# rafifmalikdzaki/Multitask-Bonetumor-yolo

Measured on AMD Instinct MI355X. Metric: images/sec at 640x640 multitask fwd (det+seg+cls) + decode/NMS/masks, higher is better.
Workload: dtype bf16; 1 GPU; configs[1]: batch-16/GPU 640x640 multitask inference (ConvNeXt-T + C2f-BiFPN + Detect/Segment/cls) + decode + per-image NMS(top-100) + mask assembly; random-init weights; batch_per_gpu=16, img=640, parallelism=dp1 (batch sharded, no data-path collective)

## Files before the change

### include/mtbt_hip.h

```cpp
#ifndef MTBT_HIP_H
#define MTBT_HIP_H

#include <stdint.h>

#ifdef __cplusplus
extern "C" {
#endif

#define MTBT_OK 0
#define MTBT_EINVAL (-1)
#define MTBT_EALIGN (-2)
#define MTBT_ELAUNCH (-3)
#define MTBT_EWORKSPACE (-4)

#define MTBT_F32 0
#define MTBT_BF16 1
#define MTBT_F16 2

#define MTBT_ACT_NONE 0
#define MTBT_ACT_SILU 1
#define MTBT_ACT_ELU 2
#define MTBT_ACT_GELU 3
#define MTBT_ACT_DSILU 5
#define MTBT_ACT_DELU 6
// ... 104 lines not shown
  int32_t act1;
  int32_t act2;
} mtbt_pw_chain_args;
int mtbt_pw_chain_nhwc(const mtbt_pw_chain_args* a, void* stream);
int mtbt_pw_chain_supported(const mtbt_pw_chain_args* a);
int mtbt_sizeof_pw_chain_args(void);

int64_t mtbt_bn_train_workspace_bytes(int64_t pixels, int C);
int mtbt_bn_train_nhwc(const void* x, void* y, const float* gamma, const float* beta, float* running_mean,
                       float* running_var, float momentum, float eps, int act, int64_t pixels, int C, int dtype,
                       void* workspace, int64_t workspace_bytes, void* stream);

int mtbt_gap_fc(const void* x, const float* w, const float* b, float* y, int N, int HW, int C,
                int nout, int dtype, void* stream);

typedef struct mtbt_decode_args {
  const float* map[3];
  int32_t h[3], w[3];
  int32_t map_pixel_stride[3];
  float stride[3];
  int32_t n_levels, N, nc, reg_max;
  int32_t xywh;
  float* boxes;
  float* scores;
  float* best_score;
  int32_t* best_label;
  float* preds_cat;
  int32_t cat_stride;
} mtbt_decode_args;

int mtbt_decode_boxes(const mtbt_decode_args* a, void* stream);

int64_t mtbt_nms_workspace_bytes(int N, int A);
int mtbt_nms_batched(const float* boxes, const float* best_score, const int32_t* best_label, int N, int A,
                     float conf_th, float iou_th, float clamp_max, int top_k, int64_t* keep_idx,
                     int32_t* keep_anchor, float* out_boxes, float* out_scores, int64_t* out_labels,
                     int32_t* counts, int32_t* n_cand, void* workspace, int64_t workspace_bytes,
                     void* stream);

typedef struct mtbt_mask_args {
  const float* protos;
  const float* coeff;
  int64_t coeff_batch_stride, coeff_k_stride, coeff_c_stride;
  const int32_t* gather_idx;
  const int32_t* counts;
  float bias;
  int32_t N, K, nm, hp, wp, Hout, Wout;
  float* logits;
  uint8_t* masks;
} mtbt_mask_args;

int mtbt_mask_assemble(const mtbt_mask_args* a, void* stream);

typedef struct mtbt_frame {
  int32_t height, width;
  float step;
  float scale;
  int32_t pitch;
  int32_t reserved;
  int64_t offset;
} mtbt_frame;

typedef struct mtbt_frame_mask_args {
  const float* protos;
  const float* coeff;
  int64_t coeff_batch_stride, coeff_k_stride, coeff_c_stride;
  const int32_t* gather_idx;
  const int32_t* counts;
  const float* boxes;
  float* boxes_frame;
  uint8_t* out;
  int64_t out_bytes;
  int32_t N, K, nm, hp, wp;
  int32_t crop;
} mtbt_frame_mask_args;

int mtbt_masks_to_frames(const mtbt_frame_mask_args* a, const mtbt_frame* frames, int n_frames, void* stream);
int mtbt_sizeof_frame_args(int which);

#define MTBT_FUSE_MAX_SOURCES 8
#define MTBT_FUSE_MAX_CANDIDATES 4096
typedef struct mtbt_box_fuse_args {
  const float* boxes[MTBT_FUSE_MAX_SOURCES];
  const float* scores[MTBT_FUSE_MAX_SOURCES];
  const int64_t* labels[MTBT_FUSE_MAX_SOURCES];
  const int32_t* counts[MTBT_FUSE_MAX_SOURCES];
  const int32_t* anchors[MTBT_FUSE_MAX_SOURCES];
  int32_t orient[MTBT_FUSE_MAX_SOURCES];
  float weight[MTBT_FUSE_MAX_SOURCES];
  int32_t n_sources, N, K, top_k;
  float img_size, iou_thr, skip_thr;
  int32_t reserved;
  float* out_boxes;
  float* out_scores;
  int64_t* out_labels;
  int32_t* out_counts;
  int32_t* n_clusters;
  int32_t* n_members;
  int32_t* lead_source;
  int32_t* lead_slot;
  int32_t* lead_anchor;
  void* workspace;
  int64_t workspace_bytes;
} mtbt_box_fuse_args;

int64_t mtbt_fuse_workspace_bytes(int n_sources, int N, int K);
// ... 423 lines not shown
```

### multitask_bonetumor_yolo_amd/_lib.py

```python
import ctypes as C
import os

_HERE = os.path.dirname(os.path.abspath(__file__))
LIB_PATH = os.path.join(_HERE, "csrc", "libmtbt_hip.so")

ABI_VERSION = 5
F32, BF16, F16 = 0, 1, 2
ACT_NONE, ACT_SILU, ACT_ELU, ACT_GELU, ACT_GELU_POLY, ACT_DSILU, ACT_DELU, ACT_DGELU, ACT_DGELU_POLY = 0, 1, 2, 3, 4, 5, 6, 7, 8
OUT_NHWC, OUT_CONVT2X2 = 0, 1
RES_ID, RES_UP_BILINEAR, RES_DOWN_MEAN, RES_UP_NEAREST, RES_MAXPOOL = 0, 1, 2, 3, 4
CONFUSION_MAX_NC = 64

ERRORS = {-1: "MTBT_EINVAL (bad argument / unsupported shape)", -2: "MTBT_EALIGN (misaligned pointer or stride)",
          -3: "MTBT_ELAUNCH (kernel launch failed)", -4: "MTBT_EWORKSPACE (workspace too small)"}


class ConvArgs(C.Structure):
    _fields_ = [
        ("x", C.c_void_p), ("w", C.c_void_p), ("y", C.c_void_p), ("scale", C.c_void_p), ("shift", C.c_void_p),
        ("res", C.c_void_p),
        ("x_batch_stride", C.c_int64), ("y_batch_stride", C.c_int64), ("res_batch_stride", C.c_int64),
        ("x_pixel_stride", C.c_int32), ("y_pixel_stride", C.c_int32), ("res_pixel_stride", C.c_int32),
        ("N", C.c_int32), ("H", C.c_int32), ("W", C.c_int32), ("C", C.c_int32), ("K", C.c_int32),
        ("R", C.c_int32), ("S", C.c_int32), ("stride", C.c_int32), ("pad", C.c_int32),
# ... 160 lines not shown


class Tile(C.Structure):
    _fields_ = [("image", C.c_int32), ("pox", C.c_int32), ("poy", C.c_int32),
                ("wx0", C.c_int32), ("wy0", C.c_int32), ("wx1", C.c_int32), ("wy1", C.c_int32),
                ("height", C.c_int32), ("width", C.c_int32), ("reserved", C.c_int32),
                ("step", C.c_float), ("scale", C.c_float), ("fox", C.c_float), ("foy", C.c_float)]


class TileMergeArgs(C.Structure):
    _fields_ = [("boxes", C.c_void_p), ("scores", C.c_void_p), ("labels", C.c_void_p), ("counts", C.c_void_p), ("anchors", C.c_void_p),
                ("tiles", C.POINTER(Tile)), ("tiles_dev", C.c_void_p), ("first", C.POINTER(C.c_int32)),
                ("N", C.c_int32), ("n_tiles", C.c_int32), ("K", C.c_int32), ("top_k", C.c_int32),
                ("metric", C.c_int32), ("class_agnostic", C.c_int32), ("thr", C.c_float), ("skip_thr", C.c_float),
                ("out_boxes", C.c_void_p), ("out_scores", C.c_void_p), ("out_labels", C.c_void_p), ("out_counts", C.c_void_p),
                ("n_members", C.c_void_p), ("lead_tile", C.c_void_p), ("lead_slot", C.c_void_p), ("lead_anchor", C.c_void_p),
                ("member_slot", C.c_void_p), ("n_left", C.c_void_p)]


class TileMaskArgs(C.Structure):
    _fields_ = [("protos", C.c_void_p), ("mc", C.c_void_p),
                ("mc_batch_stride", C.c_int64), ("mc_k_stride", C.c_int64), ("mc_c_stride", C.c_int64),
                ("anchors", C.c_void_p), ("scores", C.c_void_p), ("member_slot", C.c_void_p), ("counts", C.c_void_p), ("boxes", C.c_void_p),
                ("tiles", C.POINTER(Tile)), ("tiles_dev", C.c_void_p), ("first", C.POINTER(C.c_int32)),
                ("W", C.c_void_p), ("Ss", C.c_void_p), ("out", C.c_void_p), ("out_bytes", C.c_int64),
                ("N", C.c_int32), ("n_tiles", C.c_int32), ("K", C.c_int32), ("top_k", C.c_int32), ("Tmax", C.c_int32),
                ("nm", C.c_int32), ("hp", C.c_int32), ("wp", C.c_int32), ("crop", C.c_int32), ("reserved", C.c_int32)]


SYMBOLS = {
    "mtbt_abi_version": (C.c_int, []),
    "mtbt_sizeof_args": (C.c_int, [C.c_int]),
    "mtbt_target_arch": (C.c_char_p, []),
    "mtbt_conv2d_nhwc": (C.c_int, [C.POINTER(ConvArgs), C.c_void_p]),
    "mtbt_convt2x2_conv3x3_nhwc": (C.c_int, [C.POINTER(UpconvArgs), C.c_void_p]),
    "mtbt_stem_conv4x4_ln": (C.c_int, [C.c_void_p] * 5 + [C.c_float, C.c_void_p] + [C.c_int] * 5 + [C.c_void_p]),
    "mtbt_dwconv_nhwc": (C.c_int, [C.c_void_p] * 5 + [C.c_float, C.c_void_p, C.c_void_p, C.c_int, C.c_void_p]
                         + [C.c_int] * 6 + [C.c_void_p]),
    "mtbt_layernorm_nhwc": (C.c_int, [C.c_void_p] * 3 + [C.c_float, C.c_void_p, C.c_int64, C.c_int, C.c_int, C.c_void_p]),
    "mtbt_bifpn_fuse": (C.c_int, [C.POINTER(FuseArgs), C.c_void_p]),
    "mtbt_bifpn_node_nhwc": (C.c_int, [C.POINTER(NodeArgs), C.c_void_p]),
    "mtbt_pw_chain_nhwc": (C.c_int, [C.POINTER(PwChainArgs), C.c_void_p]),
    "mtbt_pw_chain_supported": (C.c_int, [C.POINTER(PwChainArgs)]),
    "mtbt_sizeof_pw_chain_args": (C.c_int, []),
    "mtbt_bn_train_workspace_bytes": (C.c_int64, [C.c_int64, C.c_int]),
    "mtbt_bn_train_nhwc": (C.c_int, [C.c_void_p] * 6 + [C.c_float, C.c_float, C.c_int, C.c_int64, C.c_int, C.c_int, C.c_void_p,
                                      C.c_int64, C.c_void_p]),
    "mtbt_gap_fc": (C.c_int, [C.c_void_p] * 4 + [C.c_int] * 5 + [C.c_void_p]),
    "mtbt_decode_boxes": (C.c_int, [C.POINTER(DecodeArgs), C.c_void_p]),
    "mtbt_nms_workspace_bytes": (C.c_int64, [C.c_int, C.c_int]),
    "mtbt_nms_batched": (C.c_int, [C.c_void_p] * 3 + [C.c_int, C.c_int, C.c_float, C.c_float, C.c_float, C.c_int]
                         + [C.c_void_p] * 8 + [C.c_int64, C.c_void_p]),
    "mtbt_mask_assemble": (C.c_int, [C.POINTER(MaskArgs), C.c_void_p]),
    "mtbt_loss_workspace_bytes": (C.c_int64, [C.c_int, C.c_int, C.c_int64]),
    "mtbt_multitask_loss": (C.c_int, [C.POINTER(LossArgs), C.c_void_p]),
    "mtbt_multitask_loss_grad": (C.c_int, [C.POINTER(LossArgs), C.POINTER(C.c_void_p), C.POINTER(C.c_int32), C.c_void_p, C.c_void_p, C.c_void_p]),
    "mtbt_convnext_mlp_fused": (C.c_int, [C.c_void_p] * 7 + [C.c_int64, C.c_int, C.c_void_p]),
    "mtbt_convnext_mlp_fused_dt": (C.c_int, [C.c_void_p] * 7 + [C.c_int64, C.c_int, C.c_int, C.c_void_p]),
    "mtbt_convnext_mlp_fused_train": (C.c_int, [C.c_void_p] * 8 + [C.c_int64, C.c_int, C.c_void_p]),
    "mtbt_bbox_iou_pairwise": (C.c_int, [C.c_void_p, C.c_int, C.c_void_p, C.c_int, C.c_float, C.c_void_p, C.c_void_p]),
    "mtbt_letterbox_batch": (C.c_int, [C.POINTER(RawImage), C.c_int, C.c_int, C.c_void_p, C.c_void_p, C.POINTER(C.c_double), C.c_void_p]),
    "mtbt_augment_batch": (C.c_int, [C.POINTER(RawImage), C.c_int, C.c_int, C.POINTER(C.c_int32), C.c_int, C.c_void_p, C.c_void_p, C.c_void_p, C.c_void_p]),
    "mtbt_mosaic_batch": (C.c_int, [C.POINTER(RawImage), C.c_int, C.c_int, C.POINTER(C.c_int32), C.c_int, C.POINTER(C.c_int32), C.c_void_p, C.c_void_p, C.c_void_p, C.c_void_p]),
    "mtbt_seg_confusion_workspace_bytes": (C.c_int64, [C.c_int]),
    "mtbt_seg_confusion": (C.c_int, [C.c_void_p, C.c_void_p, C.c_int, C.c_int64, C.c_void_p, C.c_void_p, C.c_void_p, C.c_int64, C.c_void_p]),
    "mtbt_conv_wgrad_workspace_bytes": (C.c_int64, [C.c_int] * 7),
    "mtbt_conv_wgrad": (C.c_int, [C.c_void_p] * 3 + [C.c_int] * 9 + [C.c_int64, C.c_int32, C.c_int64, C.c_int32, C.c_int, C.c_int, C.c_void_p,
                                  C.c_int64, C.c_void_p]),
    "mtbt_conv_wgrad_xact": (C.c_int, [C.c_void_p] * 3 + [C.c_int] * 9 + [C.c_int64, C.c_int32, C.c_int64, C.c_int32, C.c_int, C.c_int, C.c_int, C.c_void_p,
                                       C.c_int64, C.c_void_p]),
    "mtbt_conv_wgrad_bias": (C.c_int, [C.c_void_p] * 4 + [C.c_int] * 9 + [C.c_int64, C.c_int32, C.c_int64, C.c_int32, C.c_int, C.c_int, C.c_void_p,
                                       C.c_int64, C.c_void_p]),
    "mtbt_act_backward": (C.c_int, [C.c_void_p] * 3 + [C.c_int64, C.c_int, C.c_int, C.c_void_p]),
    "mtbt_channel_sum_workspace_bytes": (C.c_int64, [C.c_int64, C.c_int]),
    "mtbt_channel_sum": (C.c_int, [C.c_void_p, C.c_void_p, C.c_int64, C.c_int, C.c_int32, C.c_int32, C.c_int, C.c_void_p, C.c_int, C.c_void_p,
                                   C.c_int64, C.c_void_p]),
    "mtbt_channel_affine2": (C.c_int, [C.c_void_p] * 6 + [C.c_int64, C.c_int, C.c_int, C.c_void_p]),
    "mtbt_layernorm_backward_nhwc": (C.c_int, [C.c_void_p] * 3 + [C.c_float, C.c_void_p, C.c_void_p, C.c_int64, C.c_int, C.c_int, C.c_int, C.c_void_p]),
    "mtbt_layernorm_backward_params_workspace_bytes": (C.c_int64, [C.c_int64, C.c_int]),
    "mtbt_layernorm_backward_params_nhwc": (C.c_int, [C.c_void_p] * 3 + [C.c_float, C.c_void_p, C.c_int64, C.c_int, C.c_int, C.c_int, C.c_void_p, C.c_void_p,
                                                      C.c_int, C.c_void_p, C.c_int64, C.c_void_p]),
    "mtbt_dwconv_wgrad_workspace_bytes": (C.c_int64, [C.c_int] * 5),
    "mtbt_dwconv_wgrad": (C.c_int, [C.c_void_p] * 3 + [C.c_int] * 7 + [C.c_void_p, C.c_int64, C.c_void_p]),
    "mtbt_dwconv_wgrad_bias": (C.c_int, [C.c_void_p] * 4 + [C.c_int] * 7 + [C.c_void_p, C.c_int64, C.c_void_p]),
    "mtbt_adamw_step": (C.c_int, [C.c_void_p] * 4 + [C.c_int64] + [C.c_float] * 5 + [C.c_int64, C.c_void_p, C.c_void_p]),
    "mtbt_sgd_step": (C.c_int, [C.c_void_p] * 3 + [C.c_int64] + [C.c_float] * 4 + [C.c_int, C.c_int64, C.c_void_p, C.c_void_p]),
    "mtbt_adamw_step_ema": (C.c_int, [C.c_void_p] * 5 + [C.c_int64] + [C.c_float] * 5 + [C.c_int64, C.c_void_p, C.c_double, C.c_void_p]),
    "mtbt_sgd_step_ema": (C.c_int, [C.c_void_p] * 4 + [C.c_int64] + [C.c_float] * 4 + [C.c_int, C.c_int64, C.c_void_p, C.c_double, C.c_void_p]),
    "mtbt_ema_update": (C.c_int, [C.c_void_p, C.c_void_p, C.c_int64, C.c_double, C.c_void_p]),
    "mtbt_sumsq_workspace_bytes": (C.c_int64, []),
    "mtbt_sumsq": (C.c_int, [C.c_void_p, C.c_int64, C.c_void_p, C.c_int, C.c_void_p, C.c_int64, C.c_void_p]),
    "mtbt_clip_coef": (C.c_int, [C.c_void_p, C.c_float, C.c_void_p, C.c_void_p, C.c_void_p]),
    "mtbt_stem_conv4x4_ln_train": (C.c_int, [C.c_void_p] * 5 + [C.c_float, C.c_void_p, C.c_void_p] + [C.c_int] * 5 + [C.c_void_p]),
    "mtbt_dwconv_nhwc_train": (C.c_int, [C.c_void_p] * 5 + [C.c_float, C.c_void_p, C.c_void_p, C.c_int, C.c_void_p, C.c_void_p, C.c_void_p]
                               + [C.c_int] * 6 + [C.c_void_p]),
    "mtbt_bn_forward_nhwc": (C.c_int, [C.c_void_p, C.c_void_p, C.c_int32] + [C.c_void_p] * 4 + [C.c_float, C.c_float, C.c_int, C.c_int64, C.c_int, C.c_int,
                                       C.c_int, C.c_void_p, C.c_void_p, C.c_int64, C.c_void_p]),
    "mtbt_bn_forward_sums_nhwc": (C.c_int, [C.c_void_p, C.c_void_p, C.c_int32] + [C.c_void_p] * 4 + [C.c_float, C.c_float, C.c_int, C.c_int64, C.c_int, C.c_int,
                                            C.c_void_p, C.c_void_p, C.c_void_p, C.c_void_p]),
    "mtbt_conv_colsum_workspace_bytes": (C.c_int64, [C.c_int64, C.c_int, C.c_int]),
    "mtbt_conv_colsum_layout": (C.c_int, [C.c_void_p, C.c_void_p, C.c_void_p]),
    "mtbt_conv_kernel_choice": (C.c_int, [C.c_void_p, C.c_void_p]),
    "mtbt_conv2d_nhwc_batch": (C.c_int, [C.c_void_p, C.c_int, C.c_void_p]),
    "mtbt_conv_batch_kernel_choice": (C.c_int, [C.c_void_p, C.c_int, C.c_void_p]),
    "mtbt_dwconv3x3_mult_nhwc": (C.c_int, [C.c_void_p] * 4 + [C.c_int, C.c_void_p] + [C.c_int] * 6 + [C.c_void_p]),
    "mtbt_bn_forward_partials_nhwc": (C.c_int, [C.c_void_p, C.c_void_p, C.c_int32] + [C.c_void_p] * 4 + [C.c_float, C.c_float, C.c_int, C.c_int64, C.c_int, C.c_int,
# ... 96 lines not shown
```

### multitask_bonetumor_yolo_amd/csrc/mask_mfma.hip

```cpp
#include "common.h"

namespace {

struct MaskX4P {
  const float* protos;
  const float* coeff;
  long cbs, cks, ccs;
  const int* gather;
  const int* counts;
  float bias;
  int N, K, hp, wp, Hout, Wout;
  float* logits;
  unsigned char* masks;
  int tiles_x, tiles_y;
  int dbg;
};
#ifdef MTBT_MASK_ABLATION
#define MASK_ABL(p, bit) ((p).dbg & (bit))
#else
#define MASK_ABL(p, bit) 0
#endif

constexpr int NM = 32;
constexpr int PPITCH = NM + 1;

template <int LW, int LH, bool MASKS_ONLY>
__global__ __launch_bounds__(256) void mask_x4_kernel(const MaskX4P p) {
  constexpr int PW = LW + 2, PH = LH + 2;
  constexpr int NPX = PW * PH;
  constexpr int NPXP = (NPX + 15) / 16 * 16;
  constexpr int LPITCH = NPXP + 4;
  constexpr int SEGS = LW / 4;
  extern __shared__ __attribute__((aligned(16))) char smem[];
  float* patch = reinterpret_cast<float*>(smem);
  float* coef = patch + NPXP * PPITCH;
  float* low = coef + 16 * PPITCH;
  const int tid = threadIdx.x, lane = tid & 63, wave = tid >> 6;
  const int n = blockIdx.y;
  const int tx = blockIdx.x % p.tiles_x, ty = blockIdx.x / p.tiles_x;
  const int lx_base = tx * LW - 1, ly_base = ty * LH - 1;
  const int cnt = p.counts ? min(p.counts[n], p.K) : p.K;

  const float* pr = p.protos + (long)n * p.hp * p.wp * NM;
  for (int i = tid; i < NPXP * (NM / 4); i += 256) {
    const int px = i >> 3, c4 = i & 7;
    float4 v = make_float4(0.f, 0.f, 0.f, 0.f);
    if (px < NPX && !MASK_ABL(p, 8)) {
      const int py = px / PW, pxx = px - py * PW;
      const int ly = min(max(ly_base + py, 0), p.hp - 1), lx = min(max(lx_base + pxx, 0), p.wp - 1);
      v = *reinterpret_cast<const float4*>(pr + ((long)ly * p.wp + lx) * NM + c4 * 4);
    }
    float* d = patch + px * PPITCH + c4 * 4;
    d[0] = v.x; d[1] = v.y; d[2] = v.z; d[3] = v.w;
  }

  const int row = tid / SEGS, seg = tid % SEGS;
  const int oy = ty * (4 * LH) + row, ox0 = tx * (4 * LW) + seg * 16;
  const int iy = (row + 2) >> 2;
  const float wy1 = ((row + 2) & 3) * 0.25f + 0.125f, wy0 = 1.0f - wy1;

  float cpre[2];
  auto fetch_coef = [&](int g) {
#pragma unroll
    for (int u = 0; u < 2; ++u) {
      const int i = tid + u * 256, b = i >> 5, c = i & 31;
      float v = 0.f;
      if (g + b < cnt) {
        const long kk = p.gather ? p.gather[(long)n * p.K + g + b] : (g + b);
        v = p.coeff[(long)n * p.cbs + kk * p.cks + c * p.ccs];
      }
      cpre[u] = v;
    }
  };
  if (cnt > 0) fetch_coef(0);
  for (int g0 = 0; g0 < cnt; g0 += 16) {
#pragma unroll
    for (int u = 0; u < 2; ++u) {
      const int i = tid + u * 256;
      coef[(i >> 5) * PPITCH + (i & 31)] = cpre[u];
    }
    __syncthreads();
    if (g0 + 16 < cnt) fetch_coef(g0 + 16);
    {
      float a[8];
#pragma unroll
      for (int ks = 0; ks < 8; ++ks) a[ks] = coef[(lane & 15) * PPITCH + ks * 4 + (lane >> 4)];
      for (int pg = wave; pg < NPXP / 16 && !MASK_ABL(p, 4); pg += 4) {
        f32x4 acc = f32x4{p.bias, p.bias, p.bias, p.bias};
        const float* bp = patch + (pg * 16 + (lane & 15)) * PPITCH + (lane >> 4);
#pragma unroll
        for (int ks = 0; ks < 8; ++ks) acc = __builtin_amdgcn_mfma_f32_16x16x4f32(a[ks], bp[ks * 4], acc, 0, 0, 0);
#pragma unroll
        for (int r = 0; r < 4; ++r) low[(4 * (lane >> 4) + r) * LPITCH + pg * 16 + (lane & 15)] = acc[r];
      }
    }
    __syncthreads();
    if (oy < p.Hout && !MASK_ABL(p, 2)) {
      const int nb = min(16, cnt - g0);
      for (int b = 0; b < nb; ++b) {
        const float* r0 = low + b * LPITCH + iy * PW + seg * 4;
        const float* r1 = r0 + PW;
        float t0[6], t1[6];
#pragma unroll
        for (int c = 0; c < 6; ++c) { t0[c] = r0[c]; t1[c] = r1[c]; }
        const long obase_m = (((long)n * p.K + g0 + b) * p.Hout + oy) * p.Wout + ox0;
        if constexpr (MASKS_ONLY) {
          typedef float f2 __attribute__((ext_vector_type(2)));
          float v[6];
#pragma unroll
          for (int c = 0; c < 6; ++c) v[c] = wy0 * t0[c] + wy1 * t1[c];
          unsigned w[4] = {0u, 0u, 0u, 0u};
          if (MASK_ABL(p, 16)) {
#pragma unroll
            for (int e = 0; e < 16; ++e) {
              const int ix = (e + 2) >> 2;
              const float wx1 = ((e + 2) & 3) * 0.25f + 0.125f, wx0 = 1.0f - wx1;
              const float val = wx0 * v[ix] + wx1 * v[ix + 1];
              w[e >> 2] = __builtin_amdgcn_cvt_pk_u8_f32(fmaf(val, 0x1p100f, -0x1p76f), e & 3, w[e >> 2]);
            }
          } else
#pragma unroll
          for (int e = 0; e < 16; e += 2) {
            const int ix = (e + 2) >> 2;
            const float a1 = ((e + 2) & 3) * 0.25f + 0.125f, b1 = ((e + 3) & 3) * 0.25f + 0.125f;
            const f2 W1 = f2{a1 * 0x1p100f, b1 * 0x1p100f}, W0 = f2{(1.0f - a1) * 0x1p100f, (1.0f - b1) * 0x1p100f};
            f2 d = __builtin_elementwise_fma(W0, f2{v[ix], v[ix]}, f2{-0x1p76f, -0x1p76f});
            d = __builtin_elementwise_fma(W1, f2{v[ix + 1], v[ix + 1]}, d);
            w[e >> 2] = __builtin_amdgcn_cvt_pk_u8_f32(d.x, e & 3, w[e >> 2]);
            w[e >> 2] = __builtin_amdgcn_cvt_pk_u8_f32(d.y, (e + 1) & 3, w[e >> 2]);
          }
          if (!MASK_ABL(p, 1) || (w[0] ^ w[1] ^ w[2] ^ w[3]) == 0x12345679u) *reinterpret_cast<uint4*>(p.masks + obase_m) = uint4{w[0] & 0x01010101u, w[1] & 0x01010101u, w[2] & 0x01010101u, w[3] & 0x01010101u};
          continue;
        }
        float o[16];
#pragma unroll
        for (int e = 0; e < 16; ++e) {
          const int ix = (e + 2) >> 2;
          const float wx1 = ((e + 2) & 3) * 0.25f + 0.125f, wx0 = 1.0f - wx1;
          o[e] = wy0 * (wx0 * t0[ix] + wx1 * t0[ix + 1]) + wy1 * (wx0 * t1[ix] + wx1 * t1[ix + 1]);
        }
        const long obase = (((long)n * p.K + g0 + b) * p.Hout + oy) * p.Wout + ox0;
        if (p.logits) {
#pragma unroll
          for (int e = 0; e < 16; e += 4) *reinterpret_cast<float4*>(p.logits + obase + e) = make_float4(o[e], o[e + 1], o[e + 2], o[e + 3]);
        }
        if (p.masks) {
          unsigned w[4] = {0u, 0u, 0u, 0u};
#pragma unroll
          for (int e = 0; e < 16; ++e) w[e >> 2] |= (o[e] > 5.9604645e-8f ? 1u : 0u) << ((e & 3) * 8);
          *reinterpret_cast<uint4*>(p.masks + obase) = uint4{w[0], w[1], w[2], w[3]};
        }
      }
    }
    __syncthreads();
  }
  if (oy < p.Hout) {
    for (int k = cnt; k < p.K; ++k) {
      const long obase = (((long)n * p.K + k) * p.Hout + oy) * p.Wout + ox0;
      if (p.logits) {
#pragma unroll
        for (int e = 0; e < 16; e += 4) *reinterpret_cast<float4*>(p.logits + obase + e) = make_float4(0.f, 0.f, 0.f, 0.f);
      }
      if (p.masks) *reinterpret_cast<uint4*>(p.masks + obase) = uint4{0u, 0u, 0u, 0u};
    }
  }
}

}

template <int LW, int LH>
static int launch_mask_x4(MaskX4P& p, const mtbt_mask_args* a, hipStream_t stream) {
  static_assert(LW * LH == 256 && (LW / 4) * (4 * LH) == 256, "256 threads: one per (output row, 16-pixel segment)");
  constexpr int NPXP = ((LW + 2) * (LH + 2) + 15) / 16 * 16;
  p.tiles_x = a->Wout / (4 * LW);
  p.tiles_y = (a->Hout + 4 * LH - 1) / (4 * LH);
  const size_t lds = (size_t)(NPXP * PPITCH + 16 * PPITCH + 16 * (NPXP + 4)) * sizeof(float);
  if (!a->logits && a->masks) {
    if (int rc = mtbt_allow_lds(mask_x4_kernel<LW, LH, true>, (int)lds)) return rc;
    hipLaunchKernelGGL((mask_x4_kernel<LW, LH, true>), dim3(p.tiles_x * p.tiles_y, a->N), dim3(256), lds, stream, p);
  } else {
    if (int rc = mtbt_allow_lds(mask_x4_kernel<LW, LH, false>, (int)lds)) return rc;
    hipLaunchKernelGGL((mask_x4_kernel<LW, LH, false>), dim3(p.tiles_x * p.tiles_y, a->N), dim3(256), lds, stream, p);
  }
  MTBT_LAUNCH_CHECK();
  return MTBT_OK;
}

int mtbt_mask_x4_try(const mtbt_mask_args* a, hipStream_t stream) {
  if (a->nm != NM || a->Hout != 4 * a->hp || a->Wout != 4 * a->wp || a->Wout % 64 || a->Hout % 4) return 1;
  MaskX4P p;
  p.protos = a->protos; p.coeff = a->coeff; p.cbs = a->coeff_batch_stride; p.cks = a->coeff_k_stride; p.ccs = a->coeff_c_stride;
  p.gather = a->gather_idx; p.counts = a->counts; p.bias = a->bias;
  p.N = a->N; p.K = a->K; p.hp = a->hp; p.wp = a->wp; p.Hout = a->Hout; p.Wout = a->Wout;
  p.logits = a->logits; p.masks = a->masks;
  p.dbg = 0;
  return a->Wout % 128 == 0 ? launch_mask_x4<32, 8>(p, a, stream) : launch_mask_x4<16, 16>(p, a, stream);
}
```

### multitask_bonetumor_yolo_amd/csrc/postprocess.hip

```cpp
#include "common.h"


namespace {

struct DecodeP {
  const float* map[3];
  int h[3], w[3], ld[3], off[4];
  float stride[3];
  int n_levels, N, nc, reg_max, xywh, A;
  float* boxes;
  float* scores;
  float* best_score;
  int* best_label;
  float* preds_cat;
  int cat_stride;
};

__global__ void decode_kernel(const DecodeP p) {
  const long g = (long)blockIdx.x * 64 + (threadIdx.x >> 2);
  const int side = threadIdx.x & 3;
  const long total = (long)p.N * p.A;
  const bool live = g < total;
  const long gg = live ? g : 0;
  const int n = (int)(gg / p.A), a = (int)(gg - (long)n * p.A);
// ... 452 lines not shown
}

extern "C" int mtbt_decode_boxes(const mtbt_decode_args* a, void* stream) {
  if (!a || a->n_levels < 1 || a->n_levels > 3 || a->N <= 0 || a->nc <= 0 || a->reg_max <= 0 || a->reg_max > 64) return MTBT_EINVAL;
  DecodeP p;
  int A = 0;
  for (int l = 0; l < 3; ++l) {
    p.off[l] = A;
    if (l < a->n_levels) {
      if (!a->map[l] || a->h[l] <= 0 || a->w[l] <= 0 || a->map_pixel_stride[l] < 4 * a->reg_max + a->nc) return MTBT_EINVAL;
      p.map[l] = a->map[l]; p.h[l] = a->h[l]; p.w[l] = a->w[l]; p.ld[l] = a->map_pixel_stride[l]; p.stride[l] = a->stride[l];
      A += a->h[l] * a->w[l];
    } else { p.map[l] = nullptr; p.h[l] = p.w[l] = 1; p.ld[l] = 0; p.stride[l] = 0.f; }
  }
  p.off[3] = A;
  if (a->preds_cat && a->cat_stride < 4 + a->nc) return MTBT_EINVAL;
  p.n_levels = a->n_levels; p.N = a->N; p.nc = a->nc; p.reg_max = a->reg_max; p.xywh = a->xywh; p.A = A;
  p.boxes = a->boxes; p.scores = a->scores; p.best_score = a->best_score; p.best_label = a->best_label;
  p.preds_cat = a->preds_cat; p.cat_stride = a->cat_stride;
  const long total = (long)a->N * A;
  const long blocks = (total + 63) / 64;
  if (blocks > 0x7fffffffL) return MTBT_EINVAL;
  hipLaunchKernelGGL(decode_kernel, dim3((unsigned)blocks), dim3(256), 0, reinterpret_cast<hipStream_t>(stream), p);
  MTBT_LAUNCH_CHECK();
  return MTBT_OK;
}

extern "C" int64_t mtbt_nms_workspace_bytes(int N, int A) {
  if (N <= 0 || A <= 0) return 0;
  return (int64_t)N * nms_ws_per_image(A);
}

extern "C" int mtbt_nms_batched(const float* boxes, const float* best_score, const int32_t* best_label, int N, int A,
                                float conf_th, float iou_th, float clamp_max, int top_k, int64_t* keep_idx,
                                int32_t* keep_anchor, float* out_boxes, float* out_scores, int64_t* out_labels,
                                int32_t* counts, int32_t* n_cand, void* workspace, int64_t workspace_bytes, void* stream) {
  if (!boxes || !best_score || !keep_idx || !keep_anchor || !out_boxes || !out_scores || !out_labels || !counts || !workspace)
    return MTBT_EINVAL;
  if (N <= 0 || A <= 0 || top_k <= 0) return MTBT_EINVAL;
  if (!aligned16(boxes) || !aligned16(out_boxes) || !aligned16(workspace)) return MTBT_EALIGN;
  const long per = nms_ws_per_image(A);
  if (workspace_bytes < (int64_t)N * per) return MTBT_EWORKSPACE;
  const int P2 = pow2ceil(A);
  const int keys_in_lds = (long)P2 * 8 <= 128 * 1024 ? 1 : 0;
  const size_t lds = (size_t)NMS_KEPT_LDS * 16 + (keys_in_lds ? (size_t)P2 * 8 : 0);
  if (int rc = mtbt_allow_lds(nms_kernel, NMS_KEPT_LDS * 16 + 128 * 1024)) return rc;
  hipLaunchKernelGGL(nms_kernel, dim3(N), dim3(NMS_NT), lds, reinterpret_cast<hipStream_t>(stream), boxes, best_score, best_label, A,
                     conf_th, iou_th, clamp_max, top_k, reinterpret_cast<long long*>(keep_idx), keep_anchor, out_boxes, out_scores,
                     reinterpret_cast<long long*>(out_labels), counts, n_cand, reinterpret_cast<char*>(workspace), per, P2, keys_in_lds);
  MTBT_LAUNCH_CHECK();
  return MTBT_OK;
}

int mtbt_mask_x4_try(const mtbt_mask_args* a, hipStream_t stream);

extern "C" int mtbt_mask_assemble(const mtbt_mask_args* a, void* stream) {
  if (!a || !a->protos || !a->coeff || (!a->logits && !a->masks)) return MTBT_EINVAL;
  if (a->N <= 0 || a->K <= 0 || a->nm <= 0 || a->nm > 64 || a->nm % 4 || a->hp <= 0 || a->wp <= 0) return MTBT_EINVAL;
  if (a->Hout < a->hp || a->Wout < a->wp) return MTBT_EINVAL;
  if (a->K > 65535 || a->N > 65535) return MTBT_EINVAL;
  if (!aligned16(a->protos)) return MTBT_EALIGN;
  if (a->logits && !aligned16(a->logits)) return MTBT_EALIGN;
  if (a->masks && !aligned16(a->masks)) return MTBT_EALIGN;
  {
    const int rc = mtbt_mask_x4_try(a, reinterpret_cast<hipStream_t>(stream));
    if (rc != 1) return rc;
  }
  MaskP p;
  p.protos = a->protos; p.coeff = a->coeff; p.cbs = a->coeff_batch_stride; p.cks = a->coeff_k_stride; p.ccs = a->coeff_c_stride;
  p.gather = a->gather_idx; p.counts = a->counts; p.bias = a->bias;
  p.N = a->N; p.K = a->K; p.nm = a->nm; p.hp = a->hp; p.wp = a->wp; p.Hout = a->Hout; p.Wout = a->Wout;
  p.logits = a->logits; p.masks = a->masks;
  p.tiles_x = (a->Wout + MT - 1) / MT;
  const int tiles_y = (a->Hout + MT - 1) / MT;
  hipLaunchKernelGGL(mask_kernel, dim3(p.tiles_x * tiles_y, a->K, a->N), dim3(256), 0, reinterpret_cast<hipStream_t>(stream), p);
  MTBT_LAUNCH_CHECK();
  return MTBT_OK;
}

extern "C" int mtbt_abi_version(void) { return MTBT_ABI_VERSION; }
extern "C" int mtbt_sizeof_args(int which) {
  switch (which) {
    case 0: return (int)sizeof(mtbt_conv_args);
    case 1: return (int)sizeof(mtbt_fuse_args);
    case 2: return (int)sizeof(mtbt_decode_args);
    case 3: return (int)sizeof(mtbt_mask_args);
    case 4: return (int)sizeof(mtbt_loss_args);
    case 5: return (int)sizeof(mtbt_prep_desc);
    case 6: return (int)sizeof(mtbt_raw_image);
    case 7: return (int)sizeof(mtbt_upconv_args);
    case 8: return (int)sizeof(mtbt_node_args);
    case 9: return (int)sizeof(mtbt_box_eval_args);
    default: return -1;
  }
}
extern "C" const char* mtbt_target_arch(void) { return "gfx950"; }
```

### multitask_bonetumor_yolo_amd/postprocess.py

```python
import ctypes as C
from typing import List, Optional, Sequence

import torch

from . import _lib as L

CONF_TH, NMS_IOU, TOP_K = 0.05, 0.6, 100


def _stream(dev):
    return C.c_void_p(torch.cuda.current_stream(dev).cuda_stream)


def _need_cuda(t: torch.Tensor, what: str):
    if not t.is_cuda:
        raise RuntimeError(f"{what}: expected a CUDA/HIP tensor on an MI355X (no CPU path)")


def _nhwc_rows(t: torch.Tensor):
    assert t.dim() == 4
    t = t.float() if t.dtype != torch.float32 else t
    n, c, h, w = t.shape
    if not (t.stride(1) == 1 and t.stride(2) == w * t.stride(3) and t.stride(0) == h * w * t.stride(3)):
        t = t.contiguous(memory_format=torch.channels_last)
# ... 37 lines not shown
def detect_inference(maps, head, mc: Optional[torch.Tensor] = None) -> torch.Tensor:
    B = maps[0].N
    A = sum(m.H * m.W for m in maps)
    width = 4 + head.nc + (mc.shape[2] if mc is not None else 0)
    cat = torch.empty((B, A, width), dtype=torch.float32, device=maps[0].buf.device)
    decode_boxes([m.nchw() for m in maps], reg_max=head.reg_max, xywh=True, strides=[float(s) for s in head.stride], preds_cat=cat)
    if mc is not None:
        cat[:, :, 4 + head.nc:].copy_(mc)
    return cat.permute(0, 2, 1)


def batch_bbox_iou(boxes1: torch.Tensor, boxes2: torch.Tensor, eps: float = 1e-7) -> torch.Tensor:
    lib = L.load()
    _need_cuda(boxes1, "batch_bbox_iou")
    n, m = boxes1.shape[0], boxes2.shape[0]
    out = torch.zeros((n, m), dtype=torch.float32, device=boxes1.device)
    if n and m:
        b1, b2 = boxes1.contiguous().float(), boxes2.to(boxes1.device).contiguous().float()
        L.check(lib.mtbt_bbox_iou_pairwise(b1.data_ptr(), n, b2.data_ptr(), m, C.c_float(eps), out.data_ptr(), _stream(boxes1.device)),
                "mtbt_bbox_iou_pairwise")
    return out


def nms_batched(boxes: torch.Tensor, best_score: torch.Tensor, best_label: Optional[torch.Tensor], clamp_max: float,
                conf_th: float = CONF_TH, iou_th: float = NMS_IOU, top_k: int = TOP_K):
    lib = L.load()
    _need_cuda(boxes, "nms_batched")
    boxes = boxes.contiguous().float()
    best_score = best_score.contiguous().float()
    B, A = best_score.shape
    dev = boxes.device
    if best_label is not None:
        best_label = best_label.contiguous().to(torch.int32)
    o = {
        "keep_idx": torch.empty((B, top_k), dtype=torch.int64, device=dev),
        "keep_anchor": torch.empty((B, top_k), dtype=torch.int32, device=dev),
        "boxes": torch.empty((B, top_k, 4), dtype=torch.float32, device=dev),
        "scores": torch.empty((B, top_k), dtype=torch.float32, device=dev),
        "labels": torch.empty((B, top_k), dtype=torch.int64, device=dev),
        "counts": torch.empty((B,), dtype=torch.int32, device=dev),
        "n_cand": torch.empty((B,), dtype=torch.int32, device=dev),
    }
    wsb = lib.mtbt_nms_workspace_bytes(B, A)
    ws = torch.empty((wsb,), dtype=torch.uint8, device=dev)
    rc = lib.mtbt_nms_batched(boxes.data_ptr(), best_score.data_ptr(), best_label.data_ptr() if best_label is not None else None,
                              B, A, conf_th, iou_th, clamp_max, top_k, o["keep_idx"].data_ptr(), o["keep_anchor"].data_ptr(),
                              o["boxes"].data_ptr(), o["scores"].data_ptr(), o["labels"].data_ptr(), o["counts"].data_ptr(),
                              o["n_cand"].data_ptr(), ws.data_ptr(), wsb, _stream(dev))
    L.check(rc, "mtbt_nms_batched")
    o["_keep"] = (boxes, best_score, best_label, ws)
    return o


def _mask_call(protos, coeff, cbs, cks, ccs, gather, counts, bias, K, out_hw, want_logits, want_masks):
    lib = L.load()
    _need_cuda(protos, "mask assembly")
    pr, ld = _nhwc_rows(protos)
    B, nm, hp, wp = protos.shape
    if ld != nm:
        pr = pr.permute(0, 2, 3, 1).contiguous().permute(0, 3, 1, 2)
    dev = protos.device
    H, W = out_hw
    a = L.MaskArgs()
    a.protos, a.coeff = pr.data_ptr(), coeff.data_ptr()
    a.coeff_batch_stride, a.coeff_k_stride, a.coeff_c_stride = cbs, cks, ccs
    a.gather_idx = gather.data_ptr() if gather is not None else None
    a.counts = counts.data_ptr() if counts is not None else None
    a.bias = float(bias)
    a.N, a.K, a.nm, a.hp, a.wp, a.Hout, a.Wout = B, K, nm, hp, wp, H, W
    logits = torch.empty((B, K, H, W), dtype=torch.float32, device=dev) if want_logits else None
    masks = torch.empty((B, K, H, W), dtype=torch.bool, device=dev) if want_masks else None
    a.logits = logits.data_ptr() if logits is not None else None
    a.masks = masks.data_ptr() if masks is not None else None
    L.check(lib.mtbt_mask_assemble(C.byref(a), _stream(dev)), "mtbt_mask_assemble")
    return logits, masks


def assemble_masks(protos: torch.Tensor, mc: torch.Tensor, keep_anchor: torch.Tensor, counts: Optional[torch.Tensor],
                   out_size, want_logits: bool = False):
    assert mc.dtype == torch.float32
    keep_anchor = keep_anchor.contiguous().to(torch.int32)
    if counts is not None:
        counts = counts.contiguous().to(torch.int32)
    logits, masks = _mask_call(protos, mc, mc.stride(0), mc.stride(2), mc.stride(1), keep_anchor, counts, 0.0,
                               keep_anchor.shape[1], tuple(out_size), want_logits, True)
    return masks, logits


def proto_projector_logits(protos: torch.Tensor, weight: torch.Tensor, bias: torch.Tensor, img_size: int) -> torch.Tensor:
    w = weight.detach().reshape(-1).float().contiguous()
    logits, _ = _mask_call(protos, w, 0, 0, 1, None, None, 0.0, 1, (img_size, img_size), True, False)
    return logits.add_(bias.detach().reshape(1, 1, 1, 1).to(logits.dtype))


MAX_FRAMES = 32


def frames_of(images: Sequence[torch.Tensor], scales: Sequence[float]):
    return [(int(im.shape[0]), int(im.shape[1]), float(s)) for im, s in zip(images, scales)]


def _frame_layout(frames, K: int, up: float):
    rows, total = [], 0
    for H0, W0, scale in frames:
        H0, W0, scale = int(H0), int(W0), float(scale)
        step = C.c_float(scale / up).value if scale > 0 else 0.0
        if H0 < 1 or W0 < 1 or not 0.0 < step <= 1.0:
            raise ValueError(f"masks_to_frames: frame ({H0}, {W0}, scale {scale}) gives {step} prototype pixels per image pixel; the supported "
                             "range is 0 < scale / up <= 1, i.e. the image's long side is at least the prototype grid's (>= 160 px at S = 640)")
        pitch = 8 * ((W0 + 63) // 64)
        rows.append((H0, W0, step, C.c_float(scale).value, pitch, total))
        total = (total + K * H0 * pitch + 15) // 16 * 16
    return rows, total


def masks_to_frames(protos: torch.Tensor, mc: torch.Tensor, keep_anchor: torch.Tensor, counts: Optional[torch.Tensor],
                    boxes: Optional[torch.Tensor], frames, up: Optional[float] = None, crop: bool = False, out: Optional[torch.Tensor] = None):
    lib = L.load()
    _need_cuda(protos, "masks_to_frames")
    assert mc.dtype == torch.float32
    pr, ld = _nhwc_rows(protos)
    B, nm, hp, wp = protos.shape
    if ld != nm:
        pr = pr.permute(0, 2, 3, 1).contiguous().permute(0, 3, 1, 2)
    dev = protos.device
    keep_anchor = keep_anchor.contiguous().to(torch.int32)
    K = keep_anchor.shape[1]
    if len(frames) != B:
        raise ValueError(f"masks_to_frames: {len(frames)} frames for a batch of {B}")
    if crop and boxes is None:
        raise ValueError("masks_to_frames: crop=True needs the boxes")
    rows, total = _frame_layout(frames, K, 4.0 if up is None else float(up))
    if out is None:
        out = torch.empty((total,), dtype=torch.uint8, device=dev)
    elif out.dtype != torch.uint8 or out.dim() != 1 or not out.is_contiguous() or out.numel() < total or out.device != dev:
        raise ValueError(f"masks_to_frames: out must be a contiguous flat uint8 buffer of at least {total} bytes on {dev}")
    if counts is not None:
        counts = counts.contiguous().to(torch.int32)
# ... 381 lines not shown
```

Before: 2753 images/s.

## Add register-resident, double-buffered MFMA mask assembly kernel as default masks-only path

Adds a new masks-only mask assembly kernel. It keeps the proto patch fragments in registers, transposed with permlane swaps, instead of staging them and the coefficients in LDS. It double-buffers the low-resolution logits in LDS, so the MFMA for the next group of 16 instances overlaps with upsampling and storing the current group. It also prefetches the coefficients one group ahead. The intent is to cut LDS footprint and traffic, raise occupancy (launch bounds 256,3) and hide latency, at the cost of more register pressure and a new form-selection API path.

After: 2752 images/s (median of 4 runs). Within noise of the previous version (-0.0%).

```diff
diff --git a/include/mtbt_hip.h b/include/mtbt_hip.h
--- a/include/mtbt_hip.h
+++ b/include/mtbt_hip.h
@@ -180,6 +180,8 @@
 
 int mtbt_mask_assemble(const mtbt_mask_args* a, void* stream);
 
+int mtbt_mask_assemble_form(const mtbt_mask_args* a, int form, void* stream);
+
 typedef struct mtbt_frame {
   int32_t height, width;
   float step;
diff --git a/multitask_bonetumor_yolo_amd/_lib.py b/multitask_bonetumor_yolo_amd/_lib.py
--- a/multitask_bonetumor_yolo_amd/_lib.py
+++ b/multitask_bonetumor_yolo_amd/_lib.py
@@ -236,6 +236,7 @@
     "mtbt_nms_batched": (C.c_int, [C.c_void_p] * 3 + [C.c_int, C.c_int, C.c_float, C.c_float, C.c_float, C.c_int]
                          + [C.c_void_p] * 8 + [C.c_int64, C.c_void_p]),
     "mtbt_mask_assemble": (C.c_int, [C.POINTER(MaskArgs), C.c_void_p]),
+    "mtbt_mask_assemble_form": (C.c_int, [C.POINTER(MaskArgs), C.c_int, C.c_void_p]),
     "mtbt_loss_workspace_bytes": (C.c_int64, [C.c_int, C.c_int, C.c_int64]),
     "mtbt_multitask_loss": (C.c_int, [C.POINTER(LossArgs), C.c_void_p]),
     "mtbt_multitask_loss_grad": (C.c_int, [C.POINTER(LossArgs), C.POINTER(C.c_void_p), C.POINTER(C.c_int32), C.c_void_p, C.c_void_p, C.c_void_p]),
diff --git a/multitask_bonetumor_yolo_amd/csrc/mask_mfma.hip b/multitask_bonetumor_yolo_amd/csrc/mask_mfma.hip
--- a/multitask_bonetumor_yolo_amd/csrc/mask_mfma.hip
+++ b/multitask_bonetumor_yolo_amd/csrc/mask_mfma.hip
@@ -24,6 +24,34 @@
 constexpr int NM = 32;
 constexpr int PPITCH = NM + 1;
 
+__device__ __forceinline__ void mask_row_store(const MaskX4P& p, const float (&t0)[6], const float (&t1)[6], float wy0, float wy1, unsigned char* dst) {
+  typedef float f2 __attribute__((ext_vector_type(2)));
+  float v[6];
+#pragma unroll
+  for (int c = 0; c < 6; ++c) v[c] = wy0 * t0[c] + wy1 * t1[c];
+  unsigned w[4] = {0u, 0u, 0u, 0u};
+  if (MASK_ABL(p, 16)) {
+#pragma unroll
+    for (int e = 0; e < 16; ++e) {
+      const int ix = (e + 2) >> 2;
+      const float wx1 = ((e + 2) & 3) * 0.25f + 0.125f, wx0 = 1.0f - wx1;
+      const float val = wx0 * v[ix] + wx1 * v[ix + 1];
+      w[e >> 2] = __builtin_amdgcn_cvt_pk_u8_f32(fmaf(val, 0x1p100f, -0x1p76f), e & 3, w[e >> 2]);
+    }
+  } else
+#pragma unroll
+  for (int e = 0; e < 16; e += 2) {
+    const int ix = (e + 2) >> 2;
+    const float a1 = ((e + 2) & 3) * 0.25f + 0.125f, b1 = ((e + 3) & 3) * 0.25f + 0.125f;
+    const f2 W1 = f2{a1 * 0x1p100f, b1 * 0x1p100f}, W0 = f2{(1.0f - a1) * 0x1p100f, (1.0f - b1) * 0x1p100f};
+    f2 d = __builtin_elementwise_fma(W0, f2{v[ix], v[ix]}, f2{-0x1p76f, -0x1p76f});
+    d = __builtin_elementwise_fma(W1, f2{v[ix + 1], v[ix + 1]}, d);
+    w[e >> 2] = __builtin_amdgcn_cvt_pk_u8_f32(d.x, e & 3, w[e >> 2]);
+    w[e >> 2] = __builtin_amdgcn_cvt_pk_u8_f32(d.y, (e + 1) & 3, w[e >> 2]);
+  }
+  if (!MASK_ABL(p, 1) || (w[0] ^ w[1] ^ w[2] ^ w[3]) == 0x12345679u) *reinterpret_cast<uint4*>(dst) = uint4{w[0] & 0x01010101u, w[1] & 0x01010101u, w[2] & 0x01010101u, w[3] & 0x01010101u};
+}
+
 template <int LW, int LH, bool MASKS_ONLY>
 __global__ __launch_bounds__(256) void mask_x4_kernel(const MaskX4P p) {
   constexpr int PW = LW + 2, PH = LH + 2;
@@ -105,31 +133,7 @@
         for (int c = 0; c < 6; ++c) { t0[c] = r0[c]; t1[c] = r1[c]; }
         const long obase_m = (((long)n * p.K + g0 + b) * p.Hout + oy) * p.Wout + ox0;
         if constexpr (MASKS_ONLY) {
-          typedef float f2 __attribute__((ext_vector_type(2)));
-          float v[6];
-#pragma unroll
-          for (int c = 0; c < 6; ++c) v[c] = wy0 * t0[c] + wy1 * t1[c];
-          unsigned w[4] = {0u, 0u, 0u, 0u};
-          if (MASK_ABL(p, 16)) {
-#pragma unroll
-            for (int e = 0; e < 16; ++e) {
-              const int ix = (e + 2) >> 2;
-              const float wx1 = ((e + 2) & 3) * 0.25f + 0.125f, wx0 = 1.0f - wx1;
-              const float val = wx0 * v[ix] + wx1 * v[ix + 1];
-              w[e >> 2] = __builtin_amdgcn_cvt_pk_u8_f32(fmaf(val, 0x1p100f, -0x1p76f), e & 3, w[e >> 2]);
-            }
-          } else
-#pragma unroll
-          for (int e = 0; e < 16; e += 2) {
-            const int ix = (e + 2) >> 2;
-            const float a1 = ((e + 2) & 3) * 0.25f + 0.125f, b1 = ((e + 3) & 3) * 0.25f + 0.125f;
-            const f2 W1 = f2{a1 * 0x1p100f, b1 * 0x1p100f}, W0 = f2{(1.0f - a1) * 0x1p100f, (1.0f - b1) * 0x1p100f};
-            f2 d = __builtin_elementwise_fma(W0, f2{v[ix], v[ix]}, f2{-0x1p76f, -0x1p76f});
-            d = __builtin_elementwise_fma(W1, f2{v[ix + 1], v[ix + 1]}, d);
-            w[e >> 2] = __builtin_amdgcn_cvt_pk_u8_f32(d.x, e & 3, w[e >> 2]);
-            w[e >> 2] = __builtin_amdgcn_cvt_pk_u8_f32(d.y, (e + 1) & 3, w[e >> 2]);
-          }
-          if (!MASK_ABL(p, 1) || (w[0] ^ w[1] ^ w[2] ^ w[3]) == 0x12345679u) *reinterpret_cast<uint4*>(p.masks + obase_m) = uint4{w[0] & 0x01010101u, w[1] & 0x01010101u, w[2] & 0x01010101u, w[3] & 0x01010101u};
+          mask_row_store(p, t0, t1, wy0, wy1, p.masks + obase_m);
           continue;
         }
         float o[16];
@@ -166,16 +170,148 @@
   }
 }
 
+__device__ __forceinline__ void transpose_rows4(float (&r)[4]) {
+  unsigned u[4];
+#pragma unroll
+  for (int i = 0; i < 4; ++i) u[i] = __float_as_uint(r[i]);
+#pragma unroll
+  for (int i = 0; i < 2; ++i) {
+    const auto t = __builtin_amdgcn_permlane32_swap(u[i], u[i + 2], false, false);
+    u[i] = t[0]; u[i + 2] = t[1];
+  }
+#pragma unroll
+  for (int i = 0; i < 4; i += 2) {
+    const auto t = __builtin_amdgcn_permlane16_swap(u[i], u[i + 1], false, false);
+    u[i] = t[0]; u[i + 1] = t[1];
+  }
+#pragma unroll
+  for (int i = 0; i < 4; ++i) r[i] = __uint_as_float(u[i]);
 }
 
 template <int LW, int LH>
-static int launch_mask_x4(MaskX4P& p, const mtbt_mask_args* a, hipStream_t stream) {
+__global__ __launch_bounds__(256, 3) void mask_x4_pipe_kernel(const MaskX4P p) {
+  constexpr int PW = LW + 2, PH = LH + 2;
+  constexpr int NPX = PW * PH;
+  constexpr int NPXP = (NPX + 15) / 16 * 16;
+  constexpr int NPG = NPXP / 16;
+  constexpr int PGW = (NPG + 3) / 4;
+  constexpr int LPITCH = NPXP + 4;
+  constexpr int SEGS = LW / 4;
+  static_assert(PGW <= 6, "the resident patch fragments are sized for 6 column groups per wave");
+  extern __shared__ __attribute__((aligned(16))) char smem[];
+  float* low = reinterpret_cast<float*>(smem);
+  const int tid = threadIdx.x, lane = tid & 63;
+  const int wave = __builtin_amdgcn_readfirstlane(tid >> 6);
+  const int n = blockIdx.y;
+  const int tx = blockIdx.x % p.tiles_x, ty = blockIdx.x / p.tiles_x;
+  const int lx_base = tx * LW - 1, ly_base = ty * LH - 1;
+  const int cnt = p.counts ? min(p.counts[n], p.K) : p.K;
+
+  const int row = tid / SEGS, seg = tid % SEGS;
+  const int oy = ty * (4 * LH) + row, ox0 = tx * (4 * LW) + seg * 16;
+  const int iy = (row + 2) >> 2;
+  const float wy1 = ((row + 2) & 3) * 0.25f + 0.125f, wy0 = 1.0f - wy1;
+
+  if (cnt > 0) {
+    auto fetch_a = [&](int g, float (&a)[8]) {
+      const int b = g + (lane & 15);
+#pragma unroll
+      for (int ks = 0; ks < 8; ++ks) a[ks] = 0.f;
+      if (b < cnt) {
+        const long kk = p.gather ? p.gather[(long)n * p.K + b] : b;
+        const float* cp = p.coeff + (long)n * p.cbs + kk * p.cks + (lane >> 4) * p.ccs;
+#pragma unroll
+        for (int ks = 0; ks < 8; ++ks) a[ks] = cp[ks * 4 * p.ccs];
+      }
+    };
+    float a[8], an[8];
+    fetch_a(0, a);
+    float bf[PGW][8];
+    const float* pr = p.protos + (long)n * p.hp * p.wp * NM;
+#pragma unroll
+    for (int j = 0; j < PGW; ++j) {
+      const int px = (wave + 4 * j) * 16 + (lane & 15);
+      const bool live = px < NPX && !MASK_ABL(p, 8);
+      const int py = px / PW, pxx = px - py * PW;
+      const int ly = min(max(ly_base + py, 0), p.hp - 1), lx = min(max(lx_base + pxx, 0), p.wp - 1);
+      const float* src = pr + ((long)ly * p.wp + lx) * NM;
+      if (MASK_ABL(p, 32)) {
+#pragma unroll
+        for (int ks = 0; ks < 8; ++ks) bf[j][ks] = live ? src[ks * 4 + (lane >> 4)] : 0.f;
+        continue;
+      }
+      f32x4 v0 = f32x4{0.f, 0.f, 0.f, 0.f}, v1 = v0;
+      if (live) {
+        v0 = *reinterpret_cast<const f32x4*>(src + 8 * (lane >> 4));
+        v1 = *reinterpret_cast<const f32x4*>(src + 8 * (lane >> 4) + 4);
+      }
+      float m0[4] = {v0[0], v0[1], v0[2], v0[3]}, m1[4] = {v1[0], v1[1], v1[2], v1[3]};
+      if (wave + 4 * j < NPG) {
+        transpose_rows4(m0);
+        transpose_rows4(m1);
+      }
+#pragma unroll
+      for (int ks = 0; ks < 8; ++ks) bf[j][ks] = (ks & 1) ? m1[ks >> 1] : m0[ks >> 1];
+    }
+    auto mfma_group = [&](const float (&af)[8], float* lw) {
+#pragma unroll
+      for (int j = 0; j < PGW; ++j) {
+        const int pg = wave + 4 * j;
+        if (pg < NPG && !MASK_ABL(p, 4)) {
+          f32x4 acc = f32x4{p.bias, p.bias, p.bias, p.bias};
+#pragma unroll
+          for (int ks = 0; ks < 8; ++ks) acc = __builtin_amdgcn_mfma_f32_16x16x4f32(af[ks], bf[j][ks], acc, 0, 0, 0);
+#pragma unroll
+          for (int r = 0; r < 4; ++r) lw[(4 * (lane >> 4) + r) * LPITCH + pg * 16 + (lane & 15)] = acc[r];
+        }
+      }
+    };
+    mfma_group(a, low);
+    if (16 < cnt) fetch_a(16, an);
+    __syncthreads();
+    int buf = 0;
+    for (int g0 = 0; g0 < cnt; g0 += 16, buf ^= 1) {
+      if (g0 + 16 < cnt) {
+#pragma unroll
+        for (int ks = 0; ks < 8; ++ks) a[ks] = an[ks];
+        if (g0 + 32 < cnt) fetch_a(g0 + 32, an);
+        mfma_group(a, low + (buf ^ 1) * 16 * LPITCH);
+      }
+      if (oy < p.Hout && !MASK_ABL(p, 2)) {
+        const int nb = min(16, cnt - g0);
+        const float* lb = low + buf * 16 * LPITCH + iy * PW + seg * 4;
+        unsigned char* dst = p.masks + (((long)n * p.K + g0) * p.Hout + oy) * p.Wout + ox0;
+        for (int b = 0; b < nb; ++b) {
+          const float* r0 = lb + b * LPITCH;
+          const float* r1 = r0 + PW;
+          float t0[6], t1[6];
+#pragma unroll
+          for (int c = 0; c < 6; ++c) { t0[c] = r0[c]; t1[c] = r1[c]; }
+          mask_row_store(p, t0, t1, wy0, wy1, dst + (long)b * p.Hout * p.Wout);
+        }
+      }
+      __syncthreads();
+    }
+  }
+  if (oy < p.Hout) {
+    for (int k = cnt; k < p.K; ++k) *reinterpret_cast<uint4*>(p.masks + (((long)n * p.K + k) * p.Hout + oy) * p.Wout + ox0) = uint4{0u, 0u, 0u, 0u};
+  }
+}
+
+}
+
+constexpr int MASK_FORM_DEFAULT = 2;
+template <int LW, int LH>
+static int launch_mask_x4(MaskX4P& p, const mtbt_mask_args* a, int form, hipStream_t stream) {
   static_assert(LW * LH == 256 && (LW / 4) * (4 * LH) == 256, "256 threads: one per (output row, 16-pixel segment)");
   constexpr int NPXP = ((LW + 2) * (LH + 2) + 15) / 16 * 16;
   p.tiles_x = a->Wout / (4 * LW);
   p.tiles_y = (a->Hout + 4 * LH - 1) / (4 * LH);
   const size_t lds = (size_t)(NPXP * PPITCH + 16 * PPITCH + 16 * (NPXP + 4)) * sizeof(float);
-  if (!a->logits && a->masks) {
+  if (!a->logits && a->masks && (form ? form : MASK_FORM_DEFAULT) == 2) {
+    const size_t lds2 = (size_t)(2 * 16 * (NPXP + 4)) * sizeof(float);
+    hipLaunchKernelGGL((mask_x4_pipe_kernel<LW, LH>), dim3(p.tiles_x * p.tiles_y, a->N), dim3(256), lds2, stream, p);
+  } else if (!a->logits && a->masks) {
     if (int rc = mtbt_allow_lds(mask_x4_kernel<LW, LH, true>, (int)lds)) return rc;
     hipLaunchKernelGGL((mask_x4_kernel<LW, LH, true>), dim3(p.tiles_x * p.tiles_y, a->N), dim3(256), lds, stream, p);
   } else {
@@ -186,7 +322,7 @@
   return MTBT_OK;
 }
 
-int mtbt_mask_x4_try(const mtbt_mask_args* a, hipStream_t stream) {
+int mtbt_mask_x4_try(const mtbt_mask_args* a, int form, hipStream_t stream) {
   if (a->nm != NM || a->Hout != 4 * a->hp || a->Wout != 4 * a->wp || a->Wout % 64 || a->Hout % 4) return 1;
   MaskX4P p;
   p.protos = a->protos; p.coeff = a->coeff; p.cbs = a->coeff_batch_stride; p.cks = a->coeff_k_stride; p.ccs = a->coeff_c_stride;
@@ -194,5 +330,5 @@
   p.N = a->N; p.K = a->K; p.hp = a->hp; p.wp = a->wp; p.Hout = a->Hout; p.Wout = a->Wout;
   p.logits = a->logits; p.masks = a->masks;
   p.dbg = 0;
-  return a->Wout % 128 == 0 ? launch_mask_x4<32, 8>(p, a, stream) : launch_mask_x4<16, 16>(p, a, stream);
-}
+  return a->Wout % 128 == 0 ? launch_mask_x4<32, 8>(p, a, form, stream) : launch_mask_x4<16, 16>(p, a, form, stream);
+}
diff --git a/multitask_bonetumor_yolo_amd/csrc/postprocess.hip b/multitask_bonetumor_yolo_amd/csrc/postprocess.hip
--- a/multitask_bonetumor_yolo_amd/csrc/postprocess.hip
+++ b/multitask_bonetumor_yolo_amd/csrc/postprocess.hip
@@ -528,9 +528,10 @@
   return MTBT_OK;
 }
 
-int mtbt_mask_x4_try(const mtbt_mask_args* a, hipStream_t stream);
-
-extern "C" int mtbt_mask_assemble(const mtbt_mask_args* a, void* stream) {
+int mtbt_mask_x4_try(const mtbt_mask_args* a, int form, hipStream_t stream);
+
+extern "C" int mtbt_mask_assemble_form(const mtbt_mask_args* a, int form, void* stream) {
+  if (form < 0 || form > 2) return MTBT_EINVAL;
   if (!a || !a->protos || !a->coeff || (!a->logits && !a->masks)) return MTBT_EINVAL;
   if (a->N <= 0 || a->K <= 0 || a->nm <= 0 || a->nm > 64 || a->nm % 4 || a->hp <= 0 || a->wp <= 0) return MTBT_EINVAL;
   if (a->Hout < a->hp || a->Wout < a->wp) return MTBT_EINVAL;
@@ -538,10 +539,12 @@
   if (!aligned16(a->protos)) return MTBT_EALIGN;
   if (a->logits && !aligned16(a->logits)) return MTBT_EALIGN;
   if (a->masks && !aligned16(a->masks)) return MTBT_EALIGN;
+  if (form != 0 && (a->logits || !a->masks)) return MTBT_EINVAL;
   {
-    const int rc = mtbt_mask_x4_try(a, reinterpret_cast<hipStream_t>(stream));
+    const int rc = mtbt_mask_x4_try(a, form, reinterpret_cast<hipStream_t>(stream));
     if (rc != 1) return rc;
   }
+  if (form != 0) return MTBT_EINVAL;
   MaskP p;
   p.protos = a->protos; p.coeff = a->coeff; p.cbs = a->coeff_batch_stride; p.cks = a->coeff_k_stride; p.ccs = a->coeff_c_stride;
   p.gather = a->gather_idx; p.counts = a->counts; p.bias = a->bias;
@@ -553,6 +556,8 @@
   MTBT_LAUNCH_CHECK();
   return MTBT_OK;
 }
+
+extern "C" int mtbt_mask_assemble(const mtbt_mask_args* a, void* stream) { return mtbt_mask_assemble_form(a, 0, stream); }
 
 extern "C" int mtbt_abi_version(void) { return MTBT_ABI_VERSION; }
 extern "C" int mtbt_sizeof_args(int which) {
diff --git a/multitask_bonetumor_yolo_amd/postprocess.py b/multitask_bonetumor_yolo_amd/postprocess.py
--- a/multitask_bonetumor_yolo_amd/postprocess.py
+++ b/multitask_bonetumor_yolo_amd/postprocess.py
@@ -113,7 +113,7 @@
     return o
 
 
-def _mask_call(protos, coeff, cbs, cks, ccs, gather, counts, bias, K, out_hw, want_logits, want_masks):
+def _mask_call(protos, coeff, cbs, cks, ccs, gather, counts, bias, K, out_hw, want_logits, want_masks, form=None):
     lib = L.load()
     _need_cuda(protos, "mask assembly")
     pr, ld = _nhwc_rows(protos)
@@ -133,18 +133,21 @@
     masks = torch.empty((B, K, H, W), dtype=torch.bool, device=dev) if want_masks else None
     a.logits = logits.data_ptr() if logits is not None else None
     a.masks = masks.data_ptr() if masks is not None else None
-    L.check(lib.mtbt_mask_assemble(C.byref(a), _stream(dev)), "mtbt_mask_assemble")
+    if form is None:
+        L.check(lib.mtbt_mask_assemble(C.byref(a), _stream(dev)), "mtbt_mask_assemble")
+    else:
+        L.check(lib.mtbt_mask_assemble_form(C.byref(a), int(form), _stream(dev)), "mtbt_mask_assemble_form")
     return logits, masks
 
 
 def assemble_masks(protos: torch.Tensor, mc: torch.Tensor, keep_anchor: torch.Tensor, counts: Optional[torch.Tensor],
-                   out_size, want_logits: bool = False):
+                   out_size, want_logits: bool = False, form=None):
     assert mc.dtype == torch.float32
     keep_anchor = keep_anchor.contiguous().to(torch.int32)
     if counts is not None:
         counts = counts.contiguous().to(torch.int32)
     logits, masks = _mask_call(protos, mc, mc.stride(0), mc.stride(2), mc.stride(1), keep_anchor, counts, 0.0,
-                               keep_anchor.shape[1], tuple(out_size), want_logits, True)
+                               keep_anchor.shape[1], tuple(out_size), want_logits, True, form=form)
     return masks, logits
 
 
```
